# freudh/lbt

Hardware: AMD Instinct MI355X
Metric: train-step samples/sec, ResNet-20 CIFAR-10 8-bit DFP, 1/2/4/8 MI355X (higher is better)
Workload: dtype int8; 1 GPU; ResNet-20 CIFAR-10 8-bit DFXP W/A/G train step (fwd+bwd+SGD-momentum+range update); global_batch=128, per_gpu_batch=128, parallelism=dp1, hip_graph=True, executor=fused, grad_range=-6, loss_diverged=False

## Files before the change

### include/lbt_dfxp.h

```cpp
#ifndef LBT_DFXP_H
#define LBT_DFXP_H

#include <stdint.h>

#ifdef __cplusplus
extern "C" {
#endif

#define LBT_OK 0
#define LBT_EINVAL 1001

#define LBT_NSHARD 32
#define LBT_CSTRIDE 32

enum {
  LBT_OUT_I8 = 0,
  LBT_OUT_U8OFF = 1,
  LBT_OUT_I16 = 2,
  LBT_OUT_F32 = 3
};

typedef struct lbt_qdesc {
  const int32_t* exps;
  int32_t* counts;
// ... 174 lines not shown
  lbt_qdesc qrg; const int8_t* R; lbt_qdesc qr; const float* gb;
  lbt_qdesc qng; const int8_t* qn_codes;
  int8_t* gout; float* dout; int64_t* sums;
} lbt_bwd_branch;

typedef struct lbt_chain_bwd_a {
  const float* g; const float* y_mask; int32_t mask_from_r;
  float* gmask_out;
  lbt_bwd_branch b1, b2; int32_t has_b2;
  int64_t rows, inner; int32_t C;
} lbt_chain_bwd_a;
int lbt_bn_chain_bwd_a(const lbt_chain_bwd_a* a, void* stream);

int lbt_conv_dgrad_chain_i8(const int8_t* gq, const int8_t* wd, int32_t ksd, lbt_conv_desc d, lbt_qdesc qg,
                            lbt_qdesc qw, const float* add_src, const lbt_chain_bwd_a* a, void* stream);

int lbt_conv_dgrad2_chain_i8(const int8_t* gq, const int8_t* wd, int32_t ksd, lbt_conv_desc d, lbt_qdesc qg,
                             lbt_qdesc qw, const int8_t* gq2, const int8_t* wd2, int32_t ksd2,
                             lbt_conv_desc d2, lbt_qdesc qg2, lbt_qdesc qw2, int32_t w4,
                             const lbt_chain_bwd_a* a, void* stream);
int lbt_conv_dgrad_chain_i8w4(const int8_t* gq, const uint8_t* wd4, int32_t ksd, lbt_conv_desc d, lbt_qdesc qg,
                              lbt_qdesc qw, const float* add_src, const lbt_chain_bwd_a* a, void* stream);
int lbt_conv_dgrad_chain_wgrad_i8(const int8_t* gq, const int8_t* wd, int32_t ksd, lbt_conv_desc d, lbt_qdesc qg,
                                  lbt_qdesc qw, const float* add_src, const lbt_chain_bwd_a* a, const int8_t* xq,
                                  int32_t x_u8off, int32_t* slab, int32_t nsplit, int32_t nshard, void* stream);
int lbt_conv_dgrad_chain_wgrad_i8w4(const int8_t* gq, const uint8_t* wd4, int32_t ksd, lbt_conv_desc d,
                                    lbt_qdesc qg, lbt_qdesc qw, const float* add_src, const lbt_chain_bwd_a* a,
                                    const int8_t* xq, int32_t x_u8off, int32_t* slab, int32_t nsplit,
                                    int32_t nshard, void* stream);

typedef struct lbt_chain_bwd_b {
  const int8_t* G; lbt_qdesc qng; const int8_t* qn_codes; lbt_qdesc qn; const float* ms;
  const int64_t* sums; int64_t n;
  float* dx; int8_t* gq; lbt_qdesc qo; int64_t* gcolsum;
  int64_t rows, inner; int32_t C;
} lbt_chain_bwd_b;
int lbt_bn_chain_bwd_b(const lbt_chain_bwd_b* a, void* stream);
int lbt_conv_stem_bwd(const lbt_chain_bwd_b* b, const int16_t* x, lbt_conv_desc d, int32_t* slab, int32_t nshard,
                      void* stream);
int lbt_bn_chain_bwd_b_pair(const lbt_chain_bwd_b* a, const lbt_chain_bwd_b* b, void* stream);

typedef struct lbt_wgrad_job {
  const int8_t* xq; int32_t x_u8off; const int8_t* gq; lbt_conv_desc d;
  int32_t* slab; int32_t nsplit, nshard;
} lbt_wgrad_job;

int lbt_conv_wgrad_many_i8(const lbt_wgrad_job* jobs, int32_t njobs, void* stream);
int lbt_conv_wgrad_many_stem_i8(const lbt_wgrad_job* jobs, int32_t njobs, const lbt_chain_bwd_b* b, const int16_t* x,
                                lbt_conv_desc d, int32_t* slab, int32_t nshard, void* stream);

int lbt_conv_wgrad_many_nsplit(lbt_conv_desc d, int32_t chunks_per_wave, int32_t tap_units);
int lbt_conv_wgrad_many_blocks(lbt_conv_desc d, int32_t nsplit);
int lbt_conv_wgrad_many_slots(void);

typedef struct lbt_conv_bwd {
  lbt_chain_bwd_b b;
  const int8_t* wd; int32_t ksd; int32_t w4; lbt_conv_desc d; lbt_qdesc qw;
  const float* add_src;
  lbt_chain_bwd_a a;
  lbt_wgrad_job w;
} lbt_conv_bwd;
int lbt_conv_bwd_fused_i8(const lbt_conv_bwd* p, void* stream);

typedef struct lbt_conv_bwd2 {
  lbt_chain_bwd_b b1, bs;
  const int8_t* wd1; int32_t ksd1; const int8_t* wds; int32_t ksds; int32_t w4;
  lbt_conv_desc d1, ds; lbt_qdesc qw1, qws;
  lbt_chain_bwd_a a;
} lbt_conv_bwd2;
int lbt_conv_bwd2_fused_i8(const lbt_conv_bwd2* p, void* stream);

typedef struct lbt_conv_fwd {
  lbt_chain_fwd c;
  const int8_t* wf; int32_t ksf; int32_t w4; const int32_t* wcolsum; lbt_conv_desc d; lbt_qdesc qw;
  int8_t* yq; lbt_qdesc qout; int64_t* ychsum;
} lbt_conv_fwd;
int lbt_conv_fwd_fused_i8(const lbt_conv_fwd* p, void* stream);

int lbt_conv_fused_tile_rows(int32_t Cin, int64_t N, int32_t H);

int lbt_bn_bwd_a_wide(const float* g, lbt_qdesc qrg, const int8_t* R, const float* gamma_q, lbt_qdesc qng,
                      const int8_t* qn, int16_t* gout, float* dout, int64_t* sums, int64_t rows, int64_t inner,
                      int32_t C, void* stream);
int lbt_bn_bwd_b_wide(const int16_t* G, lbt_qdesc qng, const int8_t* qn, lbt_qdesc qn_q, const float* ms,
                      const int64_t* sums, int64_t n, float* dx, int64_t rows, int32_t C, void* stream);

int lbt_bn_bwd_a_wide_masked(const float* g, const float* g2, const float* y_mask, const uint8_t* y_bits,
                             int32_t mask_r, lbt_qdesc qr,
                             const float* gb,
                             float* gmask_out, lbt_qdesc qrg, const int8_t* R, lbt_qdesc qng, const int8_t* qn,
                             int16_t* gout, float* dout, int64_t* sums, int64_t rows, int64_t inner, int32_t C,
                             void* stream);
int lbt_bn_bwd_b_wide_q(const int16_t* G, lbt_qdesc qng, const int8_t* qn, lbt_qdesc qn_q, const float* ms,
                        const int64_t* sums, int64_t n, int16_t* gq, lbt_qdesc qo, int64_t rows, int64_t inner,
                        int32_t C, void* stream);

int lbt_bn_param_grads(const int64_t* sums, int32_t C, lbt_qdesc qrg, lbt_qdesc qr,
                       const float* gamma, float wd2, float* dgamma, float* dbeta, void* stream);


int lbt_relu_fwd(const float* x, float* y, int64_t n, void* stream);
int lbt_relu_bwd(const float* g, const float* x, float* dx, int64_t n, void* stream);
int lbt_dropout_fwd(const float* x, float* y, int64_t n, float keep, const uint64_t* step, uint64_t seed,
                    uint32_t did, int32_t relu, void* stream);
int lbt_dropout_bwd(const float* g, float* dx, int64_t n, float keep, const uint64_t* step, uint64_t seed,
                    uint32_t did, const float* relu_x, void* stream);
// ... 163 lines not shown
```

### lbt_amd/_lib.py

```python
import ctypes
import os

import torch

HERE = os.path.dirname(os.path.abspath(__file__))
LIB_PATH = os.environ.get("LBT_LIBRARY") or os.path.join(HERE, "liblbt_dfxp.so")

NSHARD = 32
STEM_WG_PIXELS = 256
CSTRIDE = 32
OUT_I8, OUT_U8OFF, OUT_I16, OUT_F32 = 0, 1, 2, 3
ABI_VERSION = 24

c_void_p, c_int32, c_int64, c_uint32, c_uint64, c_float = (
    ctypes.c_void_p, ctypes.c_int32, ctypes.c_int64, ctypes.c_uint32, ctypes.c_uint64, ctypes.c_float)


class QDesc(ctypes.Structure):
    _fields_ = [("exps", c_void_p), ("counts", c_void_p), ("step", c_void_p), ("seed", c_uint64),
                ("qid", c_uint32), ("slot", c_int32), ("bits", c_int32), ("stochastic", c_int32),
                ("noise", c_void_p)]


NO_Q = QDesc()
# ... 145 lines not shown
                ("gout", c_void_p), ("sums", c_void_p)]


class DgradBn3(ctypes.Structure):
    _fields_ = [("g2", c_void_p), ("y_bits", c_void_p), ("gmask_out", c_void_p), ("nbn", c_int32), ("pad", c_int32),
                ("bn", BnaBn * 2)]


class FSeg(ctypes.Structure):
    _fields_ = [("off", c_int64), ("n", c_int64), ("kind", c_int32), ("qx", QDesc), ("qg", QDesc), ("wd2", c_float)]


_P = c_void_p
_SIGS = {
    "lbt_abi_version": [],
    "lbt_dfxp_quantize": [_P, _P, c_int32, c_int64, c_int64, QDesc, _P, c_int32, _P],
    "lbt_dfxp_range_update": [_P, _P, _P, _P, _P, c_int32, _P, _P],
    "lbt_dfxp_counts_fold": [_P, c_int32, _P, _P],
    "lbt_dfxp_range_update_folded": [_P, _P, _P, _P, _P, c_int32, _P, _P],
    "lbt_dfxp_quantize_weight": [_P, c_int32, c_int32, c_int32, c_int32, QDesc, _P, _P, c_int32, _P, c_int32,
                                 _P, _P],
    "lbt_conv_fwd_i8": [_P, c_int32, _P, c_int32, _P, ConvDesc, QDesc, QDesc, _P, _P, QDesc, _P, _P],
    "lbt_conv_dgrad_i8": [_P, _P, c_int32, ConvDesc, QDesc, QDesc, _P, _P, _P],
    "lbt_conv_fwd_i8w4": [_P, c_int32, _P, c_int32, _P, ConvDesc, QDesc, QDesc, _P, _P, QDesc, _P, _P],
    "lbt_conv_dgrad_i8w4": [_P, _P, c_int32, ConvDesc, QDesc, QDesc, _P, _P, _P],
    "lbt_pack_int4": [_P, _P, c_int64, _P],
    "lbt_conv_fwd_igemm": [_P, c_int32, _P, c_int32, _P, ConvDesc, QDesc, QDesc, _P, _P],
    "lbt_conv_dgrad_igemm": [_P, c_int32, _P, c_int32, ConvDesc, QDesc, QDesc, _P, _P, _P],
    "lbt_conv_wgrad_igemm": [_P, _P, c_int32, ConvDesc, _P, c_int32, c_int32, _P],
    "lbt_igemm_workspace_bytes": [ConvDesc, c_int32, c_int32],
    "lbt_igemm_get_tuning": [_P],
    "lbt_igemm_set_tuning": [_P],
    "lbt_conv_fwd_igemm_q": [_P, c_int32, _P, c_int32, ConvDesc, QDesc, QDesc, _P, QDesc, _P, _P],
    "lbt_conv_fwd_igemm_ws": [_P, c_int32, _P, c_int32, _P, ConvDesc, QDesc, QDesc, _P, _P, c_int64, _P],
    "lbt_conv_dgrad_igemm_ws": [_P, c_int32, _P, c_int32, ConvDesc, QDesc, QDesc, _P, _P, _P, c_int64, _P],
    "lbt_conv_dgrad_igemm_bna": [_P, _P, c_int32, ConvDesc, QDesc, QDesc, ctypes.POINTER(DgradBna), _P, _P, c_int64,
                                 _P],
    "lbt_bn_moments": [ctypes.POINTER(BnNorm), c_int32, _P],
    "lbt_conv_dgrad_igemm_bn3": [_P, _P, c_int32, ConvDesc, QDesc, QDesc, ctypes.POINTER(DgradBn3), _P, _P, c_int64,
                                 _P],
    "lbt_conv_wgrad_igemm_store": [_P, _P, c_int32, ConvDesc, _P, c_int32, _P],
    "lbt_conv_dgrad_chain_i8w4": [_P, _P, c_int32, ConvDesc, QDesc, QDesc, _P, _P, _P],
    "lbt_conv_dgrad_chain_i8": [_P, _P, c_int32, ConvDesc, QDesc, QDesc, _P, _P, _P],
    "lbt_conv_dgrad_chain_wgrad_i8": [_P, _P, c_int32, ConvDesc, QDesc, QDesc, _P, _P, _P, c_int32, _P, c_int32,
                                      c_int32, _P],
    "lbt_conv_dgrad_chain_wgrad_i8w4": [_P, _P, c_int32, ConvDesc, QDesc, QDesc, _P, _P, _P, c_int32, _P, c_int32,
                                        c_int32, _P],
    "lbt_conv_wgrad_i8": [_P, c_int32, _P, ConvDesc, _P, c_int32, c_int32, _P],
    "lbt_conv_wgrad_many_i8": [_P, c_int32, _P],
    "lbt_conv_wgrad_many_stem_i8": [_P, c_int32, _P, _P, ConvDesc, _P, c_int32, _P],
    "lbt_conv_wgrad_many_nsplit": [ConvDesc, c_int32, c_int32],
    "lbt_conv_wgrad_many_blocks": [ConvDesc, c_int32],
    "lbt_conv_wgrad_many_slots": [],
    "lbt_conv_wgrad_reduce": [_P, c_int32, c_int32, c_int32, c_int32, _P, QDesc, QDesc, _P, c_float, _P, _P],
    "lbt_conv_fwd_generic": [_P, c_int32, _P, ConvDesc, QDesc, QDesc, _P, _P],
    "lbt_conv_dgrad_generic": [_P, _P, ConvDesc, QDesc, QDesc, _P, _P, _P],
    "lbt_conv_wgrad_generic": [_P, c_int32, _P, ConvDesc, _P, c_int32, _P],
    "lbt_conv_dgrad_generic16": [_P, _P, ConvDesc, QDesc, QDesc, _P, _P, _P],
    "lbt_conv_wgrad_generic16": [_P, c_int32, _P, ConvDesc, _P, c_int32, _P],
    "lbt_conv_wgrad_reduce64": [_P, c_int32, c_int32, c_int32, QDesc, QDesc, _P, c_float, _P, _P],
    "lbt_conv_wgrad_reduce64_many": [_P, c_int32, c_int32, _P],
    "lbt_conv_stem_fwd": [_P, _P, ConvDesc, QDesc, QDesc, _P, _P, QDesc, _P, _P],
    "lbt_conv_stem_wgrad": [_P, _P, ConvDesc, _P, c_int32, _P],
    "lbt_conv_stem_bwd": [_P, _P, ConvDesc, _P, c_int32, _P],
    "lbt_conv_bwd2_fused_i8": [_P, _P],
    "lbt_conv_fwd2_fused_i8": [_P, _P],
    "lbt_conv_wgrad_reduce_x": [_P, c_int32, c_int32, c_int32, c_int32, _P, _P, _P],
    "lbt_conv_wgrad_reduce64_x": [_P, c_int32, c_int32, c_int32, _P, _P],
    "lbt_dense_wgrad_x": [_P, _P, c_int32, c_int32, c_int32, c_int32, _P, _P],
    "lbt_bn_param_grads_x": [_P, c_int32, _P, _P, _P],
    "lbt_softmax_xent_n": [_P, _P, c_int32, c_int32, c_int32, _P, _P, _P, _P],
    "lbt_softmax_xent_wide_n": [_P, _P, c_int32, c_int32, c_int32, _P, _P, _P, _P],
    "lbt_conv_stem_wide_fwd": [_P, _P, ConvDesc, QDesc, QDesc, _P, _P],
    "lbt_stem_wide_nsplit": [ConvDesc],
    "lbt_conv_stem_wide_wgrad": [_P, c_int32, _P, c_int32, ConvDesc, _P, c_int32, _P],
    "lbt_dense_pack": [_P, c_int32, c_int32, _P, c_int32, _P, c_int32, _P],
    "lbt_flat_weight_blocks": [c_int64],
    "lbt_dfxp_quantize_weights_flat": [_P, _P, c_int32, c_int32, _P],
    "lbt_bn_bwd_a_wide_masked": [_P, _P, _P, _P, c_int32, QDesc, _P, _P, QDesc, _P, QDesc, _P, _P, _P, _P, c_int64, c_int64,
                                 c_int32, _P],
    "lbt_bn_bwd_b_wide_q": [_P, QDesc, _P, QDesc, _P, _P, c_int64, _P, QDesc, c_int64, c_int64, c_int32, _P],
    "lbt_dense_gemm": [_P, c_int32, c_int32, c_int32, _P, c_int32, c_int32, c_int32, QDesc, QDesc, _P, _P],
    "lbt_dense_wgrad": [_P, _P, c_int32, c_int32, c_int32, c_int32, QDesc, QDesc, _P, c_float, _P, _P],
    "lbt_softmax_xent_wide": [_P, _P, c_int32, c_int32, _P, _P, _P],
    "lbt_bn_chain_fwd": [_P, _P],
    "lbt_bn_chain_bwd_a": [_P, _P],
    "lbt_bn_chain_bwd_b": [_P, _P],
    "lbt_bn_chain_bwd_b_pair": [_P, _P, _P],
    "lbt_conv_fwd_pair_i8": [_P, _P, _P],
    "lbt_conv_dgrad2_chain_i8": [_P, _P, c_int32, ConvDesc, QDesc, QDesc, _P, _P, c_int32, ConvDesc, QDesc, QDesc,
                                 c_int32, _P, _P],
    "lbt_conv_bwd_fused_i8": [_P, _P],
    "lbt_conv_fwd_fused_i8": [_P, _P],
    "lbt_conv_fused_tile_rows": [c_int32, c_int64, c_int32],
    "lbt_bn_bwd_a_wide": [_P, QDesc, _P, _P, QDesc, _P, _P, _P, _P, c_int64, c_int64, c_int32, _P],
    "lbt_bn_bwd_b_wide": [_P, QDesc, _P, QDesc, _P, _P, c_int64, _P, c_int64, c_int32, _P],
    "lbt_bn_param_grads": [_P, c_int32, QDesc, QDesc, _P, c_float, _P, _P, _P],
    "lbt_relu_fwd": [_P, _P, c_int64, _P],
    "lbt_relu_bwd": [_P, _P, _P, c_int64, _P],
    "lbt_dropout_fwd": [_P, _P, c_int64, c_float, _P, c_uint64, c_uint32, c_int32, _P],
    "lbt_dropout_bwd": [_P, _P, c_int64, c_float, _P, c_uint64, c_uint32, _P, _P],
    "lbt_dropout_quantize": [_P, _P, c_int32, c_int64, c_int64, c_float, c_uint32, c_int32, QDesc, _P],
    "lbt_add": [_P, _P, _P, c_int64, _P],
    "lbt_maxpool_fwd": [_P, _P, _P, ConvDesc, _P],
    "lbt_maxpool_bwd": [_P, _P, _P, ConvDesc, _P],
    "lbt_maxpool_relu_bwd": [_P, _P, _P, _P, ConvDesc, _P],
# ... 79 lines not shown
```

### lbt_amd/csrc/conv_mfma.hip

```cpp
#include "conv_epilogue.h"
#include "chain_flags.h"
#include "conv_wgrad_body.h"
#include "lds_tr.h"
#include "stem_bwd.h"

#include <algorithm>
#include <utility>

using namespace lbt;

namespace {

constexpr int kThreads = 256;

enum { MODE_FWD = 0, MODE_DGRAD = 1 };

struct GemmArgs {
  const int8_t* a;
  const int8_t* b;
  int ks;
  int nslices;
  int a_fill;
  const int32_t* colsum;
  lbt_conv_desc d;
// ... 533 lines not shown
  return dgrad2_chain<false>(gq, wd, ksd, d, qg, qw, gq2, wd2, ksd2, d2, qg2, qw2, a, stream);
}
extern "C" int lbt_conv_dgrad_chain_i8(const int8_t* gq, const int8_t* wd, int32_t ksd, lbt_conv_desc d, lbt_qdesc qg,
                                       lbt_qdesc qw, const float* add_src, const lbt_chain_bwd_a* a, void* stream) {
  return dgrad_chain<false>(gq, wd, ksd, d, qg, qw, add_src, a, nullptr, 0, stream);
}
extern "C" int lbt_conv_dgrad_chain_i8w4(const int8_t* gq, const uint8_t* wd4, int32_t ksd, lbt_conv_desc d,
                                         lbt_qdesc qg, lbt_qdesc qw, const float* add_src, const lbt_chain_bwd_a* a,
                                         void* stream) {
  if (qw.bits > 4) return LBT_EINVAL;
  return dgrad_chain<true>(gq, (const int8_t*)wd4, ksd, d, qg, qw, add_src, a, nullptr, 0, stream);
}
extern "C" int lbt_conv_dgrad_chain_wgrad_i8(const int8_t* gq, const int8_t* wd, int32_t ksd, lbt_conv_desc d,
                                             lbt_qdesc qg, lbt_qdesc qw, const float* add_src,
                                             const lbt_chain_bwd_a* a, const int8_t* xq, int32_t x_u8off,
                                             int32_t* slab, int32_t nsplit, int32_t nshard, void* stream) {
  return dgrad_chain_wgrad<false>(gq, wd, ksd, d, qg, qw, add_src, a, xq, x_u8off, slab, nsplit, nshard, stream);
}
extern "C" int lbt_conv_dgrad_chain_wgrad_i8w4(const int8_t* gq, const uint8_t* wd4, int32_t ksd, lbt_conv_desc d,
                                               lbt_qdesc qg, lbt_qdesc qw, const float* add_src,
                                               const lbt_chain_bwd_a* a, const int8_t* xq, int32_t x_u8off,
                                               int32_t* slab, int32_t nsplit, int32_t nshard, void* stream) {
  if (qw.bits > 4) return LBT_EINVAL;
  return dgrad_chain_wgrad<true>(gq, (const int8_t*)wd4, ksd, d, qg, qw, add_src, a, xq, x_u8off, slab, nsplit,
                                 nshard, stream);
}

extern "C" int lbt_conv_wgrad_i8(const int8_t* xq, int32_t x_u8off, const int8_t* gq, lbt_conv_desc d,
                                    int32_t* slab, int32_t nsplit, int32_t nshard, void* stream) {
  WgradArgs wa;
  uint32_t blocks = 0;
  const int e = wgrad_setup(xq, x_u8off, gq, d, slab, nsplit, nshard, wa, blocks);
  if (e) return e;
  hipStream_t st = (hipStream_t)stream;
  switch (d.Cin / 16) {
    case 1: hipLaunchKernelGGL(conv_wgrad_kernel<1>, dim3(blocks), dim3(kThreads), 0, st, wa); break;
    case 2: hipLaunchKernelGGL(conv_wgrad_kernel<2>, dim3(blocks), dim3(kThreads), 0, st, wa); break;
    case 4: hipLaunchKernelGGL(conv_wgrad_kernel<4>, dim3(blocks), dim3(kThreads), 0, st, wa); break;
    case 8: hipLaunchKernelGGL(conv_wgrad_kernel<8>, dim3(blocks), dim3(kThreads), 0, st, wa); break;
    default: return LBT_EINVAL;
  }
  return (int)hipGetLastError();
}

namespace {
constexpr int kMaxWJobs = 24;
constexpr int kWgmOcc = 4;
constexpr int kWgmBufs = 2;
constexpr int kWgmBuf = 4096;
constexpr int kFW = 8;
constexpr int kWgmCpw = 16;
constexpr int kWgmMinUnits = 8;
constexpr int kWgmTapUnits = 16;
constexpr int kHaloMax = 3;
struct WgradMany {
  WgradArgs j[kMaxWJobs];
  uint32_t start[kMaxWJobs + 1];
  int32_t fast[kMaxWJobs];
  int n;
};
union WgradManyShared {
  WgradShared<1, kFW> s1;
  WgradShared<2, kFW> s2;
  int8_t stage[kFW][kWgmBufs * kWgmBuf];
  int red[kFW / 2][9 * 256];
};

int wgrad_s1_variant(const lbt_conv_desc& d, int nsplit) {
  if (d.KH != 3 || d.KW != 3 || d.SH != d.SW || (d.SH != 1 && d.SH != 2) || d.PT < 0 || d.PT > 1 || d.PL < 0 ||
      d.PL > 1 || d.Wo <= 0 || d.Wo > 64 || 64 % d.Wo || d.Ho % (64 / d.Wo))
    return 0;
  if (d.SH == 1 && (d.PT != 1 || d.PB != 1 || d.PL != 1 || d.PR != 1 || d.Ho != d.H || d.Wo != d.W)) return 0;
  const int64_t chunks = (int64_t)d.N * d.Ho * d.Wo / 64;
  if (nsplit <= 0 || chunks % nsplit) return 0;
  if ((chunks / nsplit + kFW - 1) / kFW * 64 > 65536) return 0;
  const int nhalo = ((64 / d.Wo - 1) * d.SH + 3) * ((d.Wo - 1) * d.SH + 3), nh = (nhalo + 63) / 64;
  const bool co2 = (d.Cout / 16) % 2 == 0;
  if (d.SH == 2) return (co2 && nh <= 5) ? 4 : 0;
  if (nh > kHaloMax) return 0;
  if (nh == 3) return 1;
  return co2 ? 3 : 2;
}
int wgrad_s1_nco(int variant) { return variant >= 3 ? 2 : 1; }

static __device__ __attribute__((aligned(16))) uint32_t kWgFill80[4] = {0x80808080u, 0x80808080u, 0x80808080u,
                                                                        0x80808080u};
typedef __attribute__((address_space(3))) void* wg_lds_vptr;
template <int N>
LBT_DEV void wg_vm_wait() {
  static_assert(N >= 0 && N < 64, "vmcnt");
  asm volatile("s_waitcnt vmcnt(%0)" ::"n"(N) : "memory");
}
template <int OFF>
LBT_DEV v4i wg_tr_frag(uint32_t a, uint32_t b) {
  v2i lo, hi;
  asm volatile("ds_read_b64_tr_b8 %0, %1 offset:%2" : "=v"(lo) : "v"(a), "n"(OFF) : "memory");
  asm volatile("ds_read_b64_tr_b8 %0, %1 offset:%2" : "=v"(hi) : "v"(b), "n"(OFF) : "memory");
  return v4i{lo.x, lo.y, hi.x, hi.y};
}
LBT_DEV void wg_tr_wait(v4i& a) { asm volatile("s_waitcnt lgkmcnt(0)" : "+v"(a)::"memory"); }
LBT_DEV void wg_tr_wait(v4i& a, v4i& b) { asm volatile("s_waitcnt lgkmcnt(0)" : "+v"(a), "+v"(b)::"memory"); }
LBT_DEV void wg_tr_wait(v4i& a, v4i& b, v4i& c) {
  asm volatile("s_waitcnt lgkmcnt(0)" : "+v"(a), "+v"(b), "+v"(c)::"memory");
}

template <int I>
using wg_int = std::integral_constant<int, I>;
template <class F, int... I>
LBT_DEV void wg_static_for(F&& f, std::integer_sequence<int, I...>) {
  (f(wg_int<I>{}), ...);
}

template <int NCO, int NH, int S = 1, int NB = kWgmBufs>
__device__ __forceinline__ void wgrad_s1_body(const WgradArgs& wa, uint32_t bid, WgradManyShared& sm) {
  constexpr int kBuf = kWgmBufs * kWgmBuf / NB;
  static_assert((NH + NCO) * 1024 <= kBuf && (NB == 1 || NB == kWgmBufs), "one ring buffer");
  const lbt_conv_desc& d = wa.d;
  const int H = d.H, W = d.W, Wo = d.Wo, Cin = d.Cin, Cout = d.Cout;
  const int ncs = Cin >> 4, ncog = (Cout >> 4) / NCO, nsplit = wa.nsplit;
  const int total = nsplit * ncs * ncog;
  const int xchunk = (total + 7) >> 3;
  const int u = (int)(bid & 7) * xchunk + (int)(bid >> 3);
  if (u >= total) return;
  const int split = u / (ncs * ncog), urem = u - split * (ncs * ncog);
  const int cis = urem / ncog, cog = urem - cis * ncog;
  const int lane = threadIdx.x & 63, wave = wave_id();
  const int j = lane & 15, kg = lane >> 4;
  const int RB = 64 / Wo, WR = (RB - 1) * S + 3, Wp = (Wo - 1) * S + 3, nhalo = WR * Wp;
  const int bpi = d.Ho / RB;
  const int cps = (int)((int64_t)d.N * bpi / nsplit);
  const int c0 = split * cps;
  const int nmine = cps > wave ? (cps - wave + kFW - 1) / kFW : 0;
  const int8_t* xfill = wa.x_fill ? reinterpret_cast<const int8_t*>(kWgFill80) : reinterpret_cast<const int8_t*>(zi());
  const int8_t* zero = reinterpret_cast<const int8_t*>(zi());
  int8_t* region = sm.stage[wave];
  typedef __attribute__((address_space(3))) int8_t wg_lds_i8;
// ... 78 lines not shown
            wg_static_for(
                [&](auto T) {
                  constexpr int t = decltype(T)::value;
                  v4i an = af;
                  if constexpr (t < 8) an = wg_tr_frag<kb + ((t + 1) % 3) * 16>(xa[(t + 1) / 3], xb[(t + 1) / 3]);
#pragma unroll
                  for (int c = 0; c < NCO; ++c)
                    acc[t][c] = __builtin_amdgcn_mfma_i32_16x16x64_i8(af, bf[c], acc[t][c], 0, 0, 0);
                  if constexpr (t < 8) {
                    wg_tr_wait(an);
                    af = an;
                  }
                },
                std::make_integer_sequence<int, 9>{});
            if constexpr (NB > 1) issue(k, s + k + NB);
          },
          std::make_integer_sequence<int, NB>{});
    }
    wg_vm_wait<0>();
  }
  LBT_TS(1);
  constexpr int kHalf = kFW / 2;
#pragma unroll
  for (int c = 0; c < NCO; ++c) {
    __syncthreads();
    if (wave < kHalf) {
#pragma unroll
      for (int t = 0; t < 9; ++t) *reinterpret_cast<v4i*>(&sm.red[wave][(t * 64 + lane) * 4]) = acc[t][c];
    }
    __syncthreads();
    if (wave >= kHalf) {
#pragma unroll
      for (int t = 0; t < 9; ++t) {
        v4i* q = reinterpret_cast<v4i*>(&sm.red[wave - kHalf][(t * 64 + lane) * 4]);
        *q = *q + acc[t][c];
      }
    }
    __syncthreads();
    if (c == 0) LBT_TS(2);
    int32_t* dst = wa.slab + (int64_t)(split % wa.nshard) * 9 * Cin * Cout + (int64_t)cis * 16 * Cout +
                   (cog * NCO + c) * 16;
    for (int i = threadIdx.x; i < 9 * 256; i += kFW * 64) {
      int v = 0;
#pragma unroll
      for (int w = 0; w < kHalf; ++w) v += sm.red[w][i];
      const int t = i >> 8, l = (i >> 2) & 63, ii = i & 3;
      const int ci = 4 * (l >> 4) + ii, co = l & 15;
      if (v) LBT_GADD(&dst[((int64_t)t * Cin + ci) * Cout + co], v);
    }
  }
  LBT_TS(3);
}

LBT_DEV void wgrad_many_block(const WgradMany& m, uint32_t b, WgradManyShared& sm) {
  int j = 0;
#pragma unroll 1
  while (j + 1 < m.n && b >= m.start[j + 1]) ++j;
  const WgradArgs& wa = m.j[j];
  const uint32_t rb = b - m.start[j];
#ifdef LBT_TRACE
  if (threadIdx.x == 0 && lbt_trace_buf) lbt_trace_buf[(size_t)blockIdx.x * 8 + 6] = (unsigned long long)(j + 1);
#endif
  switch (m.fast[j]) {
    case 1: wgrad_s1_body<1, 3>(wa, rb, sm); return;
    case 2: wgrad_s1_body<1, 2>(wa, rb, sm); return;
    case 3: wgrad_s1_body<2, 2>(wa, rb, sm); return;
    case 4: wgrad_s1_body<2, 5, 2, 1>(wa, rb, sm); return;
    default: break;
  }
  switch (wa.d.Cin >> 4) {
    case 1: conv_wgrad_body<1, kFW>(wa, rb, sm.s1); break;
    default: conv_wgrad_body<2, kFW>(wa, rb, sm.s2); break;
  }
}

__global__ __launch_bounds__(kFW * 64, kWgmOcc) void conv_wgrad_many_kernel(const WgradMany m) {
  __shared__ __attribute__((aligned(16))) WgradManyShared sm;
  wgrad_many_block(m, blockIdx.x, sm);
}

union WgradManyStemShared {
  WgradManyShared w;
  StemBwdShared<2> s;
};
static_assert(kFW * 64 == 2 * 256, "two stem row blocks per workgroup of the batched launch");
__global__ __launch_bounds__(kFW * 64, kWgmOcc) void conv_wgrad_many_stem_kernel(const WgradMany m,
                                                                                    const StemBwdArgs st,
                                                                                    uint32_t pairs, int stem_first) {
  __shared__ __attribute__((aligned(16))) WgradManyStemShared sm;
  const uint32_t b = blockIdx.x, nw = m.start[m.n];
  if (stem_first ? b < pairs : b >= nw) {
    stem_bwd_body<2>(st, stem_first ? b : b - nw, sm.s);
    return;
  }
  wgrad_many_block(m, stem_first ? b - pairs : b, sm.w);
}
static_assert(sizeof(WgradMany) + sizeof(StemBwdArgs) + 8 <= 4096, "kernel arguments");
static_assert(sizeof(WgradMany) <= 4096, "kernel arguments");

int wgrad_many_setup(const lbt_wgrad_job& w, WgradArgs& wa, uint32_t& blocks, int32_t& fast) {
  if (!w.slab || !w.xq || !w.gq) return LBT_EINVAL;
  const int e = wgrad_setup(w.xq, w.x_u8off, w.gq, w.d, w.slab, w.nsplit, w.nshard, wa, blocks);
  if (e) return e;
  fast = wgrad_s1_variant(w.d, w.nsplit);
  if (fast) {
    const int64_t units = (int64_t)w.nsplit * (w.d.Cin / 16) * (w.d.Cout / 16 / wgrad_s1_nco(fast));
    blocks = (uint32_t)((units + 7) / 8 * 8);
  } else if (w.d.Cin != 16 && w.d.Cin != 32) {
    return LBT_EINVAL;
  }
  return 0;
}
}

extern "C" int lbt_conv_wgrad_many_slots(void) {
  static const int cus = [] {
    int dev = 0, n = 0;
    if (hipGetDevice(&dev) != hipSuccess ||
        hipDeviceGetAttribute(&n, hipDeviceAttributeMultiprocessorCount, dev) != hipSuccess || n <= 0)
      n = 256;
    return n;
  }();
  return cus * (kWgmOcc * 4 / kFW);
}

extern "C" int lbt_conv_wgrad_many_blocks(lbt_conv_desc d, int32_t nsplit) {
  if (!desc_ok(d) || d.Cin % 16 || d.Cout % 16 || nsplit <= 0) return -LBT_EINVAL;
  const int v = wgrad_s1_variant(d, nsplit);
  if (!v && d.Cin != 16 && d.Cin != 32) return -LBT_EINVAL;
  const int64_t units = v ? (int64_t)nsplit * (d.Cin / 16) * (d.Cout / 16 / wgrad_s1_nco(v))
                          : (int64_t)nsplit * d.KH * d.KW * (d.Cout / 16);
  return units < ((int64_t)1 << 30) ? (int)((units + 7) / 8 * 8) : -LBT_EINVAL;
}

extern "C" int lbt_conv_wgrad_many_nsplit(lbt_conv_desc d, int32_t chunks_per_wave, int32_t tap_units) {
  if (!desc_ok(d) || d.Cin % 16 || d.Cout % 16) return -LBT_EINVAL;
  const int64_t P = (int64_t)d.N * d.Ho * d.Wo;
  const int v = wgrad_s1_variant(d, 1);
  if (!v) {
    const int64_t lo = (P + 65535) / 65536, taps = (int64_t)d.KH * d.KW * (d.Cout / 16);
    const int64_t want = std::max<int64_t>(1, (tap_units > 0 ? tap_units : kWgmTapUnits) / taps);
    return (int)std::max(lo, std::min(want, std::max<int64_t>(1, P / 512)));
  }
  const int64_t chunks = P / 64, units = (int64_t)(d.Cin / 16) * (d.Cout / 16 / wgrad_s1_nco(v));
  const int cpw = chunks_per_wave > 0 ? chunks_per_wave : kWgmCpw;
  int64_t ns = std::max<int64_t>(1, chunks / ((int64_t)kFW * cpw));
  if (chunks_per_wave <= 0) {
    while (ns * units < kWgmMinUnits && 2 * ns * kFW <= chunks) ns *= 2;
  }
  ns = std::max(ns, (chunks + kFW * 1024 - 1) / (kFW * 1024));
  while (chunks % ns) --ns;
  return (int)ns;
}

extern "C" int lbt_conv_wgrad_many_i8(const lbt_wgrad_job* jobs, int32_t njobs, void* stream) {
  if (njobs < 0 || (njobs > 0 && !jobs)) return LBT_EINVAL;
  for (int i = 0; i < njobs; ++i) {
    WgradArgs wa;
    uint32_t blocks = 0;
    int32_t fast = 0;
    const int e = wgrad_many_setup(jobs[i], wa, blocks, fast);
    if (e) return e;
  }
  for (int base = 0; base < njobs; base += kMaxWJobs) {
    WgradMany m{};
    const int n = njobs - base < kMaxWJobs ? njobs - base : kMaxWJobs;
    uint64_t total = 0;
    for (int i = 0; i < n; ++i) {
      uint32_t blocks = 0;
      wgrad_many_setup(jobs[base + i], m.j[i], blocks, m.fast[i]);
      m.start[i] = (uint32_t)total;
      total += blocks;
    }
    if (total >= 0x7fffffffull) return LBT_EINVAL;
    m.start[n] = (uint32_t)total;
    m.n = n;
    hipLaunchKernelGGL(conv_wgrad_many_kernel, dim3((unsigned)total), dim3(kFW * 64), 0, (hipStream_t)stream, m);
    const int rc = (int)hipGetLastError();
    if (rc) return rc;
  }
  return 0;
}

extern "C" int lbt_conv_stem_bwd(const lbt_chain_bwd_b* b, const int16_t* x, lbt_conv_desc d, int32_t* slab,
                                 int32_t nshard, void* stream);

extern "C" int lbt_conv_wgrad_many_stem_i8(const lbt_wgrad_job* jobs, int32_t njobs, const lbt_chain_bwd_b* b,
                                           const int16_t* x, lbt_conv_desc d, int32_t* slab, int32_t nshard,
                                           void* stream) {
  if (njobs < 0 || (njobs > 0 && !jobs) || !b || !x || !slab || nshard <= 0) return LBT_EINVAL;
  const int64_t M = (int64_t)d.N * d.Ho * d.Wo;
  if (M <= 0 || !stem_bwd_shape_ok(b, d)) return M <= 0 ? lbt_conv_wgrad_many_i8(jobs, njobs, stream) : LBT_EINVAL;
  const int64_t rblocks = M / kSbPixels, pairs = rblocks / 2;
  if (njobs > kMaxWJobs || rblocks % 2 || (pairs + nshard - 1) / nshard * 2 > 31) {
    const int e = lbt_conv_wgrad_many_i8(jobs, njobs, stream);
    return e ? e : lbt_conv_stem_bwd(b, x, d, slab, nshard, stream);
  }
  WgradMany m{};
// ... 51 lines not shown
```

Measured before the change: 315,600 samples/s.

## Add workgroup-cooperative wgrad kernel for stride-1 square 3x3 stages

Adds a new weight-gradient body in which a whole workgroup of eight waves shares one multi-buffered LDS ring holding halo input rows and output-gradient chunks. Waves are split across input/output channel tiles and pixel chunks, and partial sums are combined in LDS before the atomic slab update. It targets the three ResNet-20 residual-stage shapes (32x32x16, 16x16x32, 8x8x64), selected by default via a stage mask for stages 1 and 3. The split-count heuristic is also changed for these shapes to one unit per split. The aim is to cut redundant global loads and per-wave overhead in the old per-tile variants, at the cost of more LDS traffic, barriers and a cross-wave reduction.

After: 320,200 samples/s, median of 4. No clear change (+1.4%).

```diff
diff --git a/include/lbt_dfxp.h b/include/lbt_dfxp.h
--- a/include/lbt_dfxp.h
+++ b/include/lbt_dfxp.h
@@ -250,6 +250,7 @@
 int lbt_conv_wgrad_many_nsplit(lbt_conv_desc d, int32_t chunks_per_wave, int32_t tap_units);
 int lbt_conv_wgrad_many_blocks(lbt_conv_desc d, int32_t nsplit);
 int lbt_conv_wgrad_many_slots(void);
+int lbt_conv_wgrad_many_stages(int32_t mask);
 
 typedef struct lbt_conv_bwd {
   lbt_chain_bwd_b b;
diff --git a/lbt_amd/_lib.py b/lbt_amd/_lib.py
--- a/lbt_amd/_lib.py
+++ b/lbt_amd/_lib.py
@@ -221,6 +221,7 @@
     "lbt_conv_wgrad_many_nsplit": [ConvDesc, c_int32, c_int32],
     "lbt_conv_wgrad_many_blocks": [ConvDesc, c_int32],
     "lbt_conv_wgrad_many_slots": [],
+    "lbt_conv_wgrad_many_stages": [c_int32],
     "lbt_conv_wgrad_reduce": [_P, c_int32, c_int32, c_int32, c_int32, _P, QDesc, QDesc, _P, c_float, _P, _P],
     "lbt_conv_fwd_generic": [_P, c_int32, _P, ConvDesc, QDesc, QDesc, _P, _P],
     "lbt_conv_dgrad_generic": [_P, _P, ConvDesc, QDesc, QDesc, _P, _P, _P],
diff --git a/lbt_amd/csrc/conv_mfma.hip b/lbt_amd/csrc/conv_mfma.hip
--- a/lbt_amd/csrc/conv_mfma.hip
+++ b/lbt_amd/csrc/conv_mfma.hip
@@ -609,6 +609,7 @@
 constexpr int kWgmCpw = 16;
 constexpr int kWgmMinUnits = 8;
 constexpr int kWgmTapUnits = 16;
+constexpr unsigned kWgDefaultStages = 5;
 constexpr int kHaloMax = 3;
 struct WgradMany {
   WgradArgs j[kMaxWJobs];
@@ -623,6 +624,27 @@
   int red[kFW / 2][9 * 256];
 };
 
+constexpr int kWgSci[4] = {0, 8, 4, 1};
+unsigned& wgrad_wg_stages() {
+  static unsigned on = [] {
+    const char* e = getenv("LBT_WGRAD_WG");
+    if (!e) return kWgDefaultStages;
+    unsigned m = 0;
+    for (; *e; ++e)
+      if (*e >= '1' && *e <= '3') m |= 1u << (*e - '1');
+    return m;
+  }();
+  return on;
+}
+int wgrad_wg_stage(const lbt_conv_desc& d) {
+  const unsigned on = wgrad_wg_stages();
+  if (d.KH != 3 || d.KW != 3 || d.SH != 1 || d.SW != 1 || d.PT != 1 || d.PB != 1 || d.PL != 1 || d.PR != 1 ||
+      d.H != d.W || d.Ho != d.H || d.Wo != d.W || d.Cin != d.Cout)
+    return 0;
+  const int st = (d.W == 32 && d.Cin == 16) ? 1 : (d.W == 16 && d.Cin == 32) ? 2 : (d.W == 8 && d.Cin == 64) ? 3 : 0;
+  return st && ((on >> (st - 1)) & 1) ? st : 0;
+}
+
 int wgrad_s1_variant(const lbt_conv_desc& d, int nsplit) {
   if (d.KH != 3 || d.KW != 3 || d.SH != d.SW || (d.SH != 1 && d.SH != 2) || d.PT < 0 || d.PT > 1 || d.PL < 0 ||
       d.PL > 1 || d.Wo <= 0 || d.Wo > 64 || 64 % d.Wo || d.Ho % (64 / d.Wo))
@@ -630,6 +652,8 @@
   if (d.SH == 1 && (d.PT != 1 || d.PB != 1 || d.PL != 1 || d.PR != 1 || d.Ho != d.H || d.Wo != d.W)) return 0;
   const int64_t chunks = (int64_t)d.N * d.Ho * d.Wo / 64;
   if (nsplit <= 0 || chunks % nsplit) return 0;
+  if (const int st = wgrad_wg_stage(d))
+    if (chunks / nsplit % kWgSci[st] == 0 && chunks / nsplit * 64 <= 65536) return 4 + st;
   if ((chunks / nsplit + kFW - 1) / kFW * 64 > 65536) return 0;
   const int nhalo = ((64 / d.Wo - 1) * d.SH + 3) * ((d.Wo - 1) * d.SH + 3), nh = (nhalo + 63) / 64;
   const bool co2 = (d.Cout / 16) % 2 == 0;
@@ -639,6 +663,9 @@
   return co2 ? 3 : 2;
 }
 int wgrad_s1_nco(int variant) { return variant >= 3 ? 2 : 1; }
+int64_t wgrad_s1_units(const lbt_conv_desc& d, int variant) {
+  return variant > 4 ? 1 : (int64_t)(d.Cin / 16) * (d.Cout / 16 / wgrad_s1_nco(variant));
+}
 
 static __device__ __attribute__((aligned(16))) uint32_t kWgFill80[4] = {0x80808080u, 0x80808080u, 0x80808080u,
                                                                         0x80808080u};
@@ -823,6 +850,207 @@
   LBT_TS(3);
 }
 
+template <int ND, int M>
+LBT_DEV void wg_vm_wait_steps(int m) {
+  if constexpr (M == 0) {
+    wg_vm_wait<0>();
+  } else {
+    if (m >= M)
+      wg_vm_wait<ND * M>();
+    else
+      wg_vm_wait_steps<ND, M - 1>(m);
+  }
+}
+LBT_DEV void wg_barrier() {
+  asm volatile("" ::: "memory");
+  __builtin_amdgcn_s_barrier();
+  asm volatile("" ::: "memory");
+}
+
+template <int WO, int NCS, int NCO, int NCW, int SCI, int NI, int NBUF>
+__device__ __forceinline__ void wgrad_wg_body(const WgradArgs& wa, uint32_t bid, WgradManyShared& sm) {
+  constexpr int Cin = 16 * NCS, Cout = 16 * NCO;
+  constexpr int RB = 64 / WO, Wp = WO + 2, BR = SCI * RB, nhalo = (BR + 2) * Wp;
+  constexpr int BPI = WO / BR;
+  constexpr int NHP = (nhalo + 63) / 64;
+  constexpr int NXD = NCS * NHP, DI = NXD + NCO * SCI, D = NI * DI;
+  constexpr int XB = NXD * 1024, SUB = DI * 1024, BUF = NI * SUB;
+  constexpr int NDHI = (D + kFW - 1) / kFW, NDLO = D / kFW;
+  constexpr int NCG = NCO / NCW, OG = NCS * NCG, CG = kFW / OG, KC = NI * SCI / CG;
+  static_assert(64 % WO == 0 && WO % BR == 0 && NCO % NCW == 0, "whole rows, whole blocks");
+  static_assert(OG * CG == kFW && KC >= 1 && KC * CG == NI * SCI && (CG == 1 || NI == 1), "the deal of tiles and chunks");
+  static_assert(NBUF * BUF <= (int)sizeof(sm.stage) && NBUF >= 2 && NDHI * (NBUF - 2) < 64 && NDHI <= 8 && NDLO >= 1, "ring");
+  static_assert(CG == 1 || (CG / 2) * OG * 9 * 256 * 4 <= (int)sizeof(sm.red), "partials");
+  const int nsplit = wa.nsplit;
+  const int xchunk = (nsplit + 7) >> 3;
+  const int split = (int)(bid & 7) * xchunk + (int)(bid >> 3);
+  if (split >= nsplit) return;
+  const int lane = threadIdx.x & 63, wave = wave_id();
+  const int j = lane & 15, kg = lane >> 4;
+  const int og = wave / CG, cg = wave - og * CG;
+  const int csw = og / NCG, cow = (og - csw * NCG) * NCW;
+  const int nb = (int)((int64_t)wa.d.N * BPI / nsplit);
+  const int b0 = split * nb;
+  const int nsteps = (nb + NI - 1) / NI;
+  const int8_t* xfill = wa.x_fill ? reinterpret_cast<const int8_t*>(kWgFill80) : reinterpret_cast<const int8_t*>(zi());
+  const int8_t* zero = reinterpret_cast<const int8_t*>(zi());
+  int8_t* region = &sm.stage[0][0];
+  typedef __attribute__((address_space(3))) int8_t wg_lds_i8;
+  const uint32_t rbase = (uint32_t)(uintptr_t)(wg_lds_i8*)region;
+  const int qw = CG > 1 ? cg * KC : 0;
+  const int pa = 16 * kg + (j >> 1), pb = pa + 8;
+  uint32_t xa[3], xb[3];
+#pragma unroll
+  for (int r = 0; r < 3; ++r) {
+    xa[r] = rbase + (uint32_t)(csw * NHP * 1024 + ((qw * RB + pa / WO + r) * Wp + pa % WO) * 16 + 8 * (j & 1));
+    xb[r] = rbase + (uint32_t)(csw * NHP * 1024 + ((qw * RB + pb / WO + r) * Wp + pb % WO) * 16 + 8 * (j & 1));
+  }
+  const uint32_t ga = rbase + (uint32_t)(XB + cow * SCI * 1024 + (qw * 64 + pa) * 16 + 8 * (j & 1));
+  const uint32_t gb = rbase + (uint32_t)(XB + cow * SCI * 1024 + (qw * 64 + pb) * 16 + 8 * (j & 1));
+  int off[NDHI];
+  uint32_t fl = 0;
+#pragma unroll
+  for (int k = 0; k < NDHI; ++k) {
+    const int id = wave + kFW * k, rem = id % DI;
+    if (rem < NXD) {
+      const int cs = rem / NHP, t = lane + 64 * (rem - cs * NHP);
+      const int hy = t / Wp, hx = t - hy * Wp;
+      off[k] = ((hy - 1) * WO + hx - 1) * Cin + cs * 16;
+      fl |= ((uint32_t)(t < nhalo && hx >= 1 && hx <= WO) | (uint32_t)(hy < 1) << 1 | (uint32_t)(hy > BR) << 2) << (3 * k);
+    } else {
+      const int c = (rem - NXD) / SCI, q = rem - NXD - c * SCI;
+      off[k] = (q * 64 + lane) * Cout + c * 16;
+    }
+  }
+  v4i acc[9][NCW];
+#pragma unroll
+  for (int t = 0; t < 9; ++t)
+#pragma unroll
+    for (int c = 0; c < NCW; ++c) acc[t][c] = v4i{0, 0, 0, 0};
+
+  auto issue = [&](int kb, int s) {
+#pragma unroll
+    for (int k = 0; k < NDHI; ++k) {
+      const int id = wave + kFW * k;
+      if (id < D) {
+        const int ni = id / DI, rem = id - ni * DI;
+        const int bl = s * NI + ni;
+        const bool live = bl < nb;
+        const int blc = b0 + (live ? bl : nb - 1);
+        const int n = blc / BPI, pos = blc - n * BPI;
+        const int8_t* src;
+        if (rem < NXD) {
+          const int8_t* xim = wa.xq + (int64_t)(n * WO + pos * BR) * (WO * Cin);
+          const uint32_t f = fl >> (3 * k);
+          const bool ok = (f & 1) && !(pos == 0 && (f & 2)) && !(pos == BPI - 1 && (f & 4));
+          src = ok ? xim + off[k] : xfill;
+        } else {
+          src = live ? wa.gq + (int64_t)blc * (SCI * 64 * Cout) + off[k] : zero;
+        }
+        __builtin_amdgcn_global_load_lds(src, (wg_lds_vptr)(region + kb * BUF + id * 1024), 16, 0, 0);
+      }
+    }
+  };
+  const bool hi = wave + kFW * NDLO < D;
+  LBT_TS(0);
+#pragma unroll
+  for (int k = 0; k < NBUF - 1; ++k)
+    if (k < nsteps) issue(k, k);
+  for (int s0 = 0; s0 < nsteps; s0 += NBUF) {
+    wg_static_for(
+        [&](auto K) {
+          constexpr int k = decltype(K)::value, kb = k * BUF;
+          const int s = s0 + k;
+          if (s < nsteps) {
+            const int young = nsteps - 1 - s < NBUF - 2 ? nsteps - 1 - s : NBUF - 2;
+            if (hi)
+              wg_vm_wait_steps<NDHI, NBUF - 2>(young);
+            else
+              wg_vm_wait_steps<NDLO, NBUF - 2>(young);
+            wg_barrier();
+            if (s + NBUF - 1 < nsteps) issue((k + NBUF - 1) % NBUF, s + NBUF - 1);
+            wg_static_for(
+                [&](auto Q) {
+                  constexpr int kc = decltype(Q)::value;
+                  constexpr int xo = kb + (CG == 1 ? (kc / SCI) * SUB + (kc % SCI) * RB * Wp * 16 : kc * RB * Wp * 16);
+                  constexpr int go = kb + (CG == 1 ? (kc / SCI) * SUB + (kc % SCI) * 1024 : kc * 1024);
+                  v4i bf[NCW];
+                  wg_static_for(
+                      [&](auto C) { bf[decltype(C)::value] = wg_tr_frag<go + decltype(C)::value * SCI * 1024>(ga, gb); },
+                      std::make_integer_sequence<int, NCW>{});
+                  v4i af = wg_tr_frag<xo>(xa[0], xb[0]);
+                  if constexpr (NCW == 2)
+                    wg_tr_wait(bf[0], bf[1], af);
+                  else
+                    wg_tr_wait(bf[0], af);
+                  wg_static_for(
+                      [&](auto T) {
+                        constexpr int t = decltype(T)::value;
+                        v4i an = af;
+                        if constexpr (t < 8) an = wg_tr_frag<xo + ((t + 1) % 3) * 16>(xa[(t + 1) / 3], xb[(t + 1) / 3]);
+#pragma unroll
+                        for (int c = 0; c < NCW; ++c)
+                          acc[t][c] = __builtin_amdgcn_mfma_i32_16x16x64_i8(af, bf[c], acc[t][c], 0, 0, 0);
+                        if constexpr (t < 8) {
+                          wg_tr_wait(an);
+                          af = an;
+                        }
+                      },
+                      std::make_integer_sequence<int, 9>{});
+                },
+                std::make_integer_sequence<int, KC>{});
+          }
+        },
+        std::make_integer_sequence<int, NBUF>{});
+  }
+  wg_vm_wait<0>();
+  LBT_TS(1);
+  int32_t* slab = wa.slab + (int64_t)(split % wa.nshard) * 9 * Cin * Cout;
+  if constexpr (CG == 1) {
+    LBT_TS(2);
+#pragma unroll
+    for (int t = 0; t < 9; ++t)
+#pragma unroll
+      for (int c = 0; c < NCW; ++c)
+#pragma unroll
+        for (int i = 0; i < 4; ++i) {
+          const int v = acc[t][c][i];
+          if (v) LBT_GADD(&slab[(t * Cin + csw * 16 + 4 * kg + i) * Cout + (cow + c) * 16 + j], v);
+        }
+  } else {
+    constexpr int R = CG / 2;
+#pragma unroll
+    for (int c = 0; c < NCW; ++c) {
+      __syncthreads();
+      if (cg < R) {
+#pragma unroll
+        for (int t = 0; t < 9; ++t) *reinterpret_cast<v4i*>(&sm.red[cg * OG + og][(t * 64 + lane) * 4]) = acc[t][c];
+      }
+      __syncthreads();
+      if (cg >= R) {
+#pragma unroll
+        for (int t = 0; t < 9; ++t) {
+          v4i* q = reinterpret_cast<v4i*>(&sm.red[(cg - R) * OG + og][(t * 64 + lane) * 4]);
+          *q = *q + acc[t][c];
+        }
+      }
+      __syncthreads();
+      if (c == 0) LBT_TS(2);
+      for (int i = threadIdx.x; i < OG * 9 * 256; i += kFW * 64) {
+        const int o = i / (9 * 256), e = i - o * (9 * 256);
+        int v = 0;
+#pragma unroll
+        for (int w = 0; w < R; ++w) v += sm.red[w * OG + o][e];
+        const int t = e >> 8, l = (e >> 2) & 63, ii = e & 3;
+        const int ocs = o / NCG, oco = (o - ocs * NCG) * NCW + c;
+        const int ci = ocs * 16 + 4 * (l >> 4) + ii, co = oco * 16 + (l & 15);
+        if (v) LBT_GADD(&slab[(t * Cin + ci) * Cout + co], v);
+      }
+    }
+  }
+  LBT_TS(3);
+}
+
 LBT_DEV void wgrad_many_block(const WgradMany& m, uint32_t b, WgradManyShared& sm) {
   int j = 0;
 #pragma unroll 1
@@ -837,6 +1065,9 @@
     case 2: wgrad_s1_body<1, 2>(wa, rb, sm); return;
     case 3: wgrad_s1_body<2, 2>(wa, rb, sm); return;
     case 4: wgrad_s1_body<2, 5, 2, 1>(wa, rb, sm); return;
+    case 5: wgrad_wg_body<32, 1, 1, 1, 8, 1, 3>(wa, rb, sm); return;
+    case 6: wgrad_wg_body<16, 2, 2, 2, 4, 1, 3>(wa, rb, sm); return;
+    case 7: wgrad_wg_body<8, 4, 4, 2, 1, 2, 2>(wa, rb, sm); return;
     default: break;
   }
   switch (wa.d.Cin >> 4) {
@@ -875,7 +1106,7 @@
   if (e) return e;
   fast = wgrad_s1_variant(w.d, w.nsplit);
   if (fast) {
-    const int64_t units = (int64_t)w.nsplit * (w.d.Cin / 16) * (w.d.Cout / 16 / wgrad_s1_nco(fast));
+    const int64_t units = (int64_t)w.nsplit * wgrad_s1_units(w.d, fast);
     blocks = (uint32_t)((units + 7) / 8 * 8);
   } else if (w.d.Cin != 16 && w.d.Cin != 32) {
     return LBT_EINVAL;
@@ -895,11 +1126,18 @@
   return cus * (kWgmOcc * 4 / kFW);
 }
 
+extern "C" int lbt_conv_wgrad_many_stages(int32_t mask) {
+  unsigned& on = wgrad_wg_stages();
+  const int old = (int)on;
+  if (mask >= 0) on = (unsigned)mask & 7u;
+  return old;
+}
+
 extern "C" int lbt_conv_wgrad_many_blocks(lbt_conv_desc d, int32_t nsplit) {
   if (!desc_ok(d) || d.Cin % 16 || d.Cout % 16 || nsplit <= 0) return -LBT_EINVAL;
   const int v = wgrad_s1_variant(d, nsplit);
   if (!v && d.Cin != 16 && d.Cin != 32) return -LBT_EINVAL;
-  const int64_t units = v ? (int64_t)nsplit * (d.Cin / 16) * (d.Cout / 16 / wgrad_s1_nco(v))
+  const int64_t units = v ? (int64_t)nsplit * wgrad_s1_units(d, v)
                           : (int64_t)nsplit * d.KH * d.KW * (d.Cout / 16);
   return units < ((int64_t)1 << 30) ? (int)((units + 7) / 8 * 8) : -LBT_EINVAL;
 }
@@ -907,14 +1145,27 @@
 extern "C" int lbt_conv_wgrad_many_nsplit(lbt_conv_desc d, int32_t chunks_per_wave, int32_t tap_units) {
   if (!desc_ok(d) || d.Cin % 16 || d.Cout % 16) return -LBT_EINVAL;
   const int64_t P = (int64_t)d.N * d.Ho * d.Wo;
+  const int cpw = chunks_per_wave > 0 ? chunks_per_wave : kWgmCpw;
+  const int64_t chunks = P / 64;
+  if (const int st = wgrad_wg_stage(d)) {
+    const int64_t units = st == 1 ? 1 : st == 2 ? 2 : 8;
+    int64_t ns = std::max<int64_t>(1, chunks * units / ((int64_t)kFW * cpw));
+    if (chunks_per_wave <= 0)
+      while (ns < kWgmMinUnits && 2 * ns * kWgSci[st] <= chunks) ns *= 2;
+    ns = std::min(ns, chunks / kWgSci[st]);
+    for (int64_t n = ns; n >= 1; --n)
+      if (wgrad_s1_variant(d, (int)n) > 4) return (int)n;
+    for (int64_t n = ns + 1; n <= chunks; ++n)
+      if (wgrad_s1_variant(d, (int)n) > 4) return (int)n;
+    return -LBT_EINVAL;
+  }
   const int v = wgrad_s1_variant(d, 1);
   if (!v) {
     const int64_t lo = (P + 65535) / 65536, taps = (int64_t)d.KH * d.KW * (d.Cout / 16);
     const int64_t want = std::max<int64_t>(1, (tap_units > 0 ? tap_units : kWgmTapUnits) / taps);
     return (int)std::max(lo, std::min(want, std::max<int64_t>(1, P / 512)));
   }
-  const int64_t chunks = P / 64, units = (int64_t)(d.Cin / 16) * (d.Cout / 16 / wgrad_s1_nco(v));
-  const int cpw = chunks_per_wave > 0 ? chunks_per_wave : kWgmCpw;
+  const int64_t units = wgrad_s1_units(d, v);
   int64_t ns = std::max<int64_t>(1, chunks / ((int64_t)kFW * cpw));
   if (chunks_per_wave <= 0) {
     while (ns * units < kWgmMinUnits && 2 * ns * kFW <= chunks) ns *= 2;
```
